# nvpro-samples/vk_gltf_renderer

Hardware: AMD Instinct MI355X
Metric: Msamples/s (and ms/frame @ fixed spp) 1080p & 4K, 1/2/4/8 MI355X (higher is better)
Workload: dtype f32

## Files before the change

vk_gltf_renderer_amd/csrc/device/mi_pt_api.hip:

```cpp
#include <hip/hip_runtime.h>

#include <algorithm>
#include <chrono>
#include <cstdlib>
#include <cmath>
#include <cstdio>
#include <cstring>
#include <memory>
#include <string>
#include <vector>

#include "mi_pt.h"
#include "bvh_refit.h"
#include "material_patch.h"
#include "pt_build.h"
#include "pt_bvh.h"
#include "pt_deform.h"
#include "pt_kernels.h"

namespace {

thread_local std::string g_lastError;

int fail(int code, const std::string& msg)
// ... 37 lines not shown
    ptr   = nullptr;
    count = 0;
  }
  ~DevBuf() { release(); }
};

enum TimedKernel { TK_GENERATE, TK_TRACE, TK_SORT, TK_SHADE, TK_SHADOW, TK_ACCUM, TK_PRIMARY, TK_SHADE_FIRST, TK_COUNT };

}

struct RunSwitches
{
  int    packetInterval = 1;
  int    sortMode       = 2;
  bool   noPacket       = false;
  bool   stateBySlot    = false;
  bool   traceSpans     = false;
  int    overlapUpTo    = 32;
  int    overlapMinTris = 200000;
  bool   noPlanes       = false;
  bool   noOpaqueTris   = false;
  bool   noQuads        = false;
  bool   shadowFarFirst = true;
  int    reinsert       = 16;
  int    reinsertUpdate = 0;
  int    reinsertRounds = 4;
  float  splitFactor    = 4.0f;
  int    splitMaxDepth  = 8;
  float  splitMinShare  = 0.1f;
  bool   collapseGreedy = false;
  bool   collapseBad    = false;
  bool   hostCollapse   = false;
  bool   coreTex        = true;
  int    maxItersDiag   = 0;
  int    failBuildAt    = 0;
  bool   candPoolSet    = false;
  size_t candPool       = 0;
  void   read()
  {
    auto flag = [](const char* n) { const char* e = getenv(n); return e != nullptr; };
    auto num  = [](const char* n, int d) { const char* e = getenv(n); return e ? atoi(e) : d; };
    packetInterval = num("MI_PT_PACKET_INTERVAL", 1);
    sortMode       = num("MI_PT_SORT", 2);
    noPacket       = flag("MI_PT_NO_PACKET");
    stateBySlot    = flag("MI_PT_STATE_BY_SLOT");
    traceSpans     = flag("MI_PT_TRACE_SPANS");
    overlapUpTo    = num("MI_PT_OVERLAP", 32);
    overlapMinTris = num("MI_PT_OVERLAP_MIN_TRIS", 200000);
    noPlanes       = flag("MI_PT_DIAG_NO_PLANES");
    noOpaqueTris   = flag("MI_PT_DIAG_NO_OPAQUE_TRIS");
    noQuads        = flag("MI_PT_DIAG_NO_QUADS");
    shadowFarFirst = num("MI_PT_SHADOW_FAR_FIRST", 1) != 0;
    reinsert       = std::max(0, num("MI_PT_REINSERT", 16));
    reinsertUpdate = std::max(0, num("MI_PT_REINSERT_UPDATE", 0));
    reinsertRounds = std::max(1, num("MI_PT_REINSERT_ROUNDS", 4));
    if(const char* e = getenv("MI_PT_SPLIT"))
      splitFactor = std::max(0.0f, float(atof(e)));
    if(const char* e = getenv("MI_PT_SPLIT_MIN_SHARE"))
      splitMinShare = std::max(0.0f, float(atof(e)));
    splitMaxDepth  = std::min(std::max(0, num("MI_PT_SPLIT_DEPTH", 8)), 10);
    if(const char* e = getenv("MI_PT_COLLAPSE"))
    {
      collapseGreedy = strcmp(e, "greedy") == 0;
      collapseBad    = !collapseGreedy && strcmp(e, "sah") != 0;
    }
    hostCollapse   = flag("MI_PT_HOST_COLLAPSE");
    maxItersDiag   = num("MI_PT_DIAG_MAX_ITERS", 0);
    coreTex        = num("MI_PT_CORE_TEX", 1) != 0;
    failBuildAt    = num("MI_PT_DIAG_FAIL_BUILD", 0);
    if(const char* e = getenv("MI_PT_DIAG_CAND_POOL"))
    {
      candPoolSet = true;
      candPool    = size_t(strtoull(e, nullptr, 10));
    }
  }
};

struct MiPt
{
  int device = 0;
  int numCUs = 256;
  RunSwitches sw;
  int accelBuilds = 0;
  int               frameQueueDepth = 1;
  int               pendingFrames   = 0;
  MiPathtraceParams pendingFirst{};
  void*             pendingStream   = nullptr;
  DevBuf<MiGltfShadeMaterial> materials;
  DevBuf<MiGltfTextureInfo>   texInfos;
  DevBuf<pt::DevTexRef>       texRefs;
  DevBuf<pt::DevCoreTex>      coreTex;
  DevBuf<MiGltfRenderNode>    nodes;
  DevBuf<pt::DevPrim>         prims;
  DevBuf<MiGltfLight>         lights;
  DevBuf<pt::DevTexture>      textures;
  DevBuf<uchar4>              texels;
  DevBuf<uint4>               texQuads;
  DevBuf<uint8_t>             geometry;
  DevBuf<uint8_t>             instFlags;
  DevBuf<float>               srgbLut;
  DevBuf<float4>              envPixels;
// ... 1869 lines not shown
  c.fc.height    = pt->height;
  c.fc.tileSize  = pt->tileSize;
  c.fc.tileShift = 0;
  while((1 << c.fc.tileShift) < pt->tileSize)
    ++c.fc.tileShift;
  c.fc.numSlots  = pt->numSlots;
  c.fc.numFrames = numFrames;
  pt::divideMagic(uint32_t(std::max(numFrames, 2)), c.fc.framesMagic, c.fc.framesShift);
  c.fc.slotLayout = numFrames % 64 == 0 ? 1 : 0;
  c.fc.stateInQueue = (!pt->sw.stateBySlot && !(pt->frameInfo.flags & MI_SCENE_INFINITE_PLANE_SHADOW_CATCHER)) ? 1 : 0;
  const bool guides = (params->flags & MI_PT_USE_OPTIX_DENOISER) != 0;
  if(int rc = ensureOptionalPathArrays(pt, c.fc.stateInQueue == 0, params->numSamples > 1, guides, (pt->frameInfo.flags & MI_SCENE_INFINITE_PLANE_SHADOW_CATCHER) != 0))
    return rc;
  c.paths        = pt->paths;
  {
    const bool stateBySlot = c.fc.stateInQueue == 0, multiSample = params->numSamples > 1;
    if(!(stateBySlot || multiSample))
      c.paths.misc = nullptr;
    if(!stateBySlot)
      c.paths.throughput = nullptr;
    if(!multiSample)
      c.paths.pixelSum = nullptr;
  }
  pt->accumFrames   = float(params->totalSamples) / float(params->numSamples) + float(numFrames);
  if(guides && (params->totalSamples == 0 || pt->momentFrames == pt->accumFrames - float(numFrames)))
    pt->momentFrames = pt->accumFrames;
  else if(!guides || params->totalSamples == 0)
    pt->momentFrames = 0.0f;
  if(!guides)
  {
    c.paths.guideAlbedo = nullptr;
    c.paths.guideNormal = nullptr;
  }
  c.queues           = pt->queues;
  if(!(pt->frameInfo.flags & MI_SCENE_INFINITE_PLANE_SHADOW_CATCHER))
    c.queues.shadow.aux2 = nullptr;
  c.ownedTiles       = pt->ownedTiles.ptr;
  c.stats            = pt->stats.ptr;
  c.stream           = stream;
  c.persistentBlocks = unsigned(pt->numCUs) * 8u;
  c.hasAlpha         = pt->hasAlpha;
  c.hasAlphaClosest  = c.hasAlpha && pt->hasAlphaTest;
  c.visualization    = pt->frameInfo.visualization > MI_VIZ_RENDERED && pt->frameInfo.visualization < MI_VIZ_COUNT;
  if(pt->frameInfo.visualization == MI_VIZ_OPACITY_MICROMAP)
    c.hasAlphaClosest = false;
  c.hasTransmissive  = pt->hasTransmissive;
  c.simpleMaterials  = pt->simpleMaterials;
  c.wide             = pt->wide;
  c.collectCounters  = pt->collectCounters;
  {
    c.sortMode = pt->sw.sortMode;
  }
  if(pt->sceneDevDirty)
  {
    HIP_TRY(hipDeviceSynchronize());
    HIP_TRY(pt->sceneDev.upload(&pt->scene, 1));
    pt->sceneDevDirty = false;
  }
  if(!pt->fcHost)
  {
    HIP_TRY(hipHostMalloc(reinterpret_cast<void**>(&pt->fcHost), sizeof(pt::FrameConsts) * MiPt::FC_RING, hipHostMallocDefault));
    HIP_TRY(pt->fcRing.alloc(MiPt::FC_RING));
    for(hipEvent_t& e : pt->fcDone)
      HIP_TRY(hipEventCreateWithFlags(&e, hipEventDisableTiming));
  }
  const unsigned fcSlot = pt->fcCursor++ % unsigned(MiPt::FC_RING);
// ... 654 lines not shown
```

vk_gltf_renderer_amd/csrc/device/pt_kernels.hip:

```cpp
#include <hip/hip_runtime.h>
#include <hip/hip_fp16.h>

#ifndef MI_PT_EXACT_FP
#define PT_FAST_SHADING_MATH 1
#endif
#include "pt_kernels.h"
#include "pt_shading.h"
#include "pt_bvh.h"
#include "pt_bvh8.h"
#include "pt_packet.h"
#include "pt_feed.h"
#include "pt_visualize.h"

namespace pt {

namespace {

constexpr int TRACE_BLOCK = 1024;
#ifndef NODE_CACHE_EXTRA
#define NODE_CACHE_EXTRA 0
#endif
constexpr int NODE_CACHE  = 712 + NODE_CACHE_EXTRA;
constexpr int NODE_CACHE_ALPHA = 504 + NODE_CACHE_EXTRA;
constexpr int SEL_BLOCK   = 256;
// ... 305 lines not shown
    const uint32_t pos   = (chunk % NSUB) * Q.subCap + (chunk / NSUB) * QCHUNK + (slot % QCHUNK);
    Q.active[0].slot[pos] = cp.valid ? slot : QUEUE_DEAD;
    if(cp.valid)
    {
      Q.active[0].org[pos] = make_float4(cp.origin.x, cp.origin.y, cp.origin.z, 0.0f);
      Q.active[0].dir[pos] = make_float4(cp.direction.x, cp.direction.y, cp.direction.z, __uint_as_float(cp.seed));
      if(fc.stateInQueue)
        Q.active[0].misc[pos] = make_float4(0.0f, __uint_as_float(PF_ALIVE), __uint_as_float(cp.seed), 0.0f);
    }
  }
  if(blockIdx.x == 0 && threadIdx.x < NSUB)
  {
    const uint32_t numChunks = batchSlots / QCHUNK;
    Q.counters[QC_PAIR0 + 2 * threadIdx.x] = QCHUNK * (numChunks / NSUB + (threadIdx.x < numChunks % NSUB ? 1u : 0u));
  }
  if(blockIdx.x == 0 && threadIdx.x < 8)
    Q.counters[QC_HEADS_TRACE + threadIdx.x] = 0;
  (void)sc;
}

#ifdef TRACE_PROFILE
__device__ unsigned long long g_traceProf[20];
__device__ unsigned long long g_shadowProf[16];
#define PROF_T() __builtin_amdgcn_s_memtime()
#define PROF_ADD(i, t0) profAcc[i] += PROF_T() - (t0)
#define PROF_CNT(i, n) profCnt[i] += (unsigned long long)(n)
#else
#define PROF_T() 0ull
#define PROF_ADD(i, t0) (void)(t0)
#define PROF_CNT(i, n) (void)0
#endif

#ifdef SHADE_PROFILE
__device__ unsigned long long g_shadeProf[20];
#define SPROF_BEGIN() const unsigned long long sprofT0_ = __builtin_amdgcn_s_memtime(); const int sprofLanes_ = __popcll(__ballot(true))
#define SPROF_END(r)                                                                                                             \
  do                                                                                                                             \
  {                                                                                                                              \
    if(!FIRST)                                                                                                                   \
    {                                                                                                                            \
      const unsigned long long dt_ = __builtin_amdgcn_s_memtime() - sprofT0_;                                                   \
      if(laneId() == uint32_t(__ffsll((long long)__ballot(true)) - 1))                                                          \
      {                                                                                                                          \
        atomicAdd(&g_shadeProf[2 * (r)], dt_);                                                                                   \
        atomicAdd(&g_shadeProf[2 * (r) + 1], dt_ * (unsigned long long)sprofLanes_);                                             \
      }                                                                                                                          \
    }                                                                                                                            \
  } while(0)
#else
#define SPROF_BEGIN() (void)0
#define SPROF_END(r) (void)0
#endif

#ifndef REFILL_IDLE_LANES
#define REFILL_IDLE_LANES 16
#endif
#ifndef TRI_PHASE_LANES_N
#define TRI_PHASE_LANES_N 24
#endif
constexpr int TRI_PHASE_LANES      = TRI_PHASE_LANES_N;
constexpr int TRI_PHASE_EXIT_LANES = 10;
#ifndef TRI_ROUND_LANES
#define TRI_ROUND_LANES 20
#endif
#ifndef TRI_ROUND_LANE_CAP_N
#define TRI_ROUND_LANE_CAP_N 4
#endif
// ... 1723 lines not shown
    out[i] = makeShadeRecord(sc, sc.tris[i]);
}

__global__ void __launch_bounds__(256) k_texture_quads(const uint32_t* __restrict__ texels, uint4* __restrict__ quads, uint32_t offset, int w, int h, int wrapS, int wrapT)
{
  const uint32_t i = blockIdx.x * 256u + threadIdx.x;
  if(i >= uint32_t(w) * uint32_t(h))
    return;
  const int x = int(i % uint32_t(w)), y = int(i / uint32_t(w));
  const int x1 = wrapS == MI_WRAP_CLAMP_TO_EDGE ? min(x + 1, w - 1) : (x + 1 == w ? 0 : x + 1);
  const int y1 = wrapT == MI_WRAP_CLAMP_TO_EDGE ? min(y + 1, h - 1) : (y + 1 == h ? 0 : y + 1);
  const uint32_t* L = texels + offset;
  quads[offset + i] = make_uint4(L[uint32_t(y) * uint32_t(w) + uint32_t(x)], L[uint32_t(y) * uint32_t(w) + uint32_t(x1)],
                                 L[uint32_t(y1) * uint32_t(w) + uint32_t(x)], L[uint32_t(y1) * uint32_t(w) + uint32_t(x1)]);
}

__global__ void k_reset_counters(uint32_t* counters)
{
  for(int i = threadIdx.x; i < QC_COUNT; i += blockDim.x)
    counters[i] = 0;
}

}

void launchBuildAlphaRecords(const DevScene& scene, uint32_t numTris, DevAlphaTri* out, hipStream_t s)
{
  if(numTris)
    hipLaunchKernelGGL(k_alpha_records, dim3((numTris + 255) / 256), dim3(256), 0, s, scene, numTris, out);
}
void dumpTraceProfile()
{
#ifdef SHADE_PROFILE
  {
    unsigned long long h[20] = {};
    (void)hipDeviceSynchronize();
    (void)hipMemcpyFromSymbol(h, HIP_SYMBOL(g_shadeProf), sizeof(h));
    const double tot = h[18] ? double(h[18]) : 1.0;
    const char*  names[9] = {"entry + hit state", "material + textures", "sampleLights", "bsdfEvaluate", "bsdfSample", "(unused)", "miss (inline / listed)", "append + stores", "finishMisses"};
    fprintf(stderr, "[mi_pt shade profile] later-bounce k_shade: round ticks %.4g, lanes with an entry %.1f\n", tot, h[18] ? double(h[19]) / double(h[18]) : 0.0);
    for(int r = 0; r < 9; ++r)
      if(h[2 * r])
        fprintf(stderr, "[mi_pt shade profile]   %-24s %5.1f %% of the round's wave time, %5.1f lanes inside\n", names[r], 100.0 * double(h[2 * r]) / tot,
                r == 8 ? 0.0 : double(h[2 * r + 1]) / double(h[2 * r]));
  }
#endif
#ifdef TRACE_PROFILE
  unsigned long long h[20] = {};
  (void)hipDeviceSynchronize();
  (void)hipMemcpyFromSymbol(h, HIP_SYMBOL(g_traceProf), sizeof(h));
  const double tot = double(h[3]) > 0 ? double(h[3]) : 1.0;
  fprintf(stderr, "[mi_pt trace profile] feed split: start-ray (waits for the prefetch) %.1f%% take %.1f%% issue %.1f%%\n", 100.0 * h[5] / tot, 100.0 * h[6] / tot,
          100.0 * h[7] / tot);
  fprintf(stderr, "[mi_pt trace profile] waves %llu total ticks %.4g: feed %.1f%% node %.1f%% tri %.1f%% other %.1f%%\n", h[4], tot, 100.0 * h[0] / tot,
          100.0 * h[1] / tot, 100.0 * h[2] / tot, 100.0 * (tot - h[0] - h[1] - h[2]) / tot);
  fprintf(stderr, "[mi_pt trace profile] triangle rounds: test (permutes, intersection, alpha) %.1f%% gather %.1f%% of total; alpha rounds %.1f%% of total (%llu rounds)\n",
          100.0 * h[16] / tot, 100.0 * h[17] / tot, 100.0 * h[18] / tot, h[19]);
  unsigned long long g[16] = {};
  (void)hipMemcpyFromSymbol(g, HIP_SYMBOL(g_shadowProf), sizeof(g));
  const double st = double(g[5]) > 0 ? double(g[5]) : 1.0;
  const auto   pr = [](unsigned long long a, unsigned long long b) { return b ? double(a) / double(b) : 0.0; };
  fprintf(stderr, "[mi_pt shadow profile] waves %llu total ticks %.4g: feed %.1f%% node %.1f%% tri %.1f%% alpha %.1f%% finish %.1f%% other %.1f%%\n", g[6], st,
          100.0 * g[0] / st, 100.0 * g[1] / st, 100.0 * g[2] / st, 100.0 * g[3] / st, 100.0 * g[4] / st, 100.0 * (st - g[0] - g[1] - g[2] - g[3] - g[4]) / st);
  fprintf(stderr, "[mi_pt shadow profile] outer iterations %llu (%.1f idle lanes each), inner iterations %llu (%.1f active lanes, %.1f visiting), alpha rounds %llu (%.1f entries)\n",
          g[8], pr(g[9], g[8]), g[10], pr(g[11], g[10]), pr(g[12], g[10]), g[13], pr(g[14], g[13]));
  const auto per = [](unsigned long long a, unsigned long long b) { return b ? double(a) / double(b) : 0.0; };
  fprintf(stderr, "[mi_pt trace profile] lanes: %.1f of 64 visit per node step (%llu steps, %.1f blocked); %.1f test per triangle round (%llu rounds in %llu phases); "
                  "%.1f idle at each of %llu refills\n",
          per(h[9], h[8]), h[8], per(h[15], h[8]), per(h[11], h[10]), h[10], h[14], per(h[13], h[12]), h[12]);
#endif
// ... 193 lines not shown
```

vk_gltf_renderer_amd/csrc/device/pt_scene.h:

```cpp
#pragma once
#include <hip/hip_runtime.h>
#include <stdint.h>

#include "mi_pt.h"
#include "pt_math.h"

namespace pt {

struct DevTexture
{
  uint32_t levelOffset[16];
  uint16_t width, height;
  uint8_t  numLevels;
  uint8_t  srgb;
  uint8_t  magFilter, minFilter, mipmapMode, wrapS, wrapT;
  uint8_t  _pad[5];
};

struct DevTexRef
{
  float    uv[6];
  uint32_t level0;
  uint16_t width, height;
  uint8_t  numLevels, srgb, magFilter, minFilter, mipmapMode, wrapS, wrapT, texCoord;
// ... 111 lines not shown
  const float*               srgbLut;
  int                        numMaterials, numTextures, numLights, numNodes;
  int                        envWidth, envHeight;
  int                        numTris;
  int                        bvh8NumNodes;
  int                        bvhRoot;
  int                        packetInterval;
  uint32_t                   shadowOctFlip;
};

struct SkyPrecomp
{
  float sunDir[3], cosS;
  float thetaS, tS, T, cosTs;
  float sunE[3], Yz;
  float xz, yz, sunRadius, coneAngle;
  float coneOneMinusCos, omega, denY, denX;
  float denYy, pad0, pad1, pad2;
  float cY[5], cX[5], cYy[5], pad3;
};
struct FrameConsts
{
  MiSceneFrameInfo        frameInfo;
  MiSkyPhysicalParameters sky;
  const SkyPrecomp*       skyPre;
  MiPathtraceParams       pc;
  int                     width, height;
  int                     tileSize, tileShift;
  int                     numSlots;
  int                     numFrames;
  uint32_t                framesMagic, framesShift;
  int                     slotLayout;
  int                     stateInQueue;
};

inline void divideMagic(uint32_t d, uint32_t& magic, uint32_t& shift)
{
  uint32_t k = 31;
  while(!(d >> k))
    --k;
  if((d & (d - 1u)) == 0u)
  {
    magic = 0x80000000u;
    shift = k - 1u;
    return;
  }
  const unsigned long long p = 1ull << (32 + k);
  magic                      = uint32_t((p + d - 1ull) / d);
  shift                      = k;
}

#if defined(__HIPCC__)
template <class T, class I>
__device__ __forceinline__ const T& gat(const T* table, I i)
{
  return *(const T*)((const __attribute__((address_space(1))) T*)table + i);
}
template <class T>
__device__ __forceinline__ const T& uniformConst(const T& r)
{
  const unsigned long long p = reinterpret_cast<unsigned long long>(&r);
  const uint32_t           lo = uint32_t(__builtin_amdgcn_readfirstlane(int(uint32_t(p)))), hi = uint32_t(__builtin_amdgcn_readfirstlane(int(uint32_t(p >> 32))));
  const unsigned long long u  = (unsigned long long)lo | ((unsigned long long)hi << 32);
  return *(const T*)(const __attribute__((address_space(4))) T*)u;
}
#else
// ... 109 lines not shown
```

vk_gltf_renderer_amd/csrc/device/pt_shade_body.h:

```cpp
  const DevScene&    sc = uniformConst(*scp);
  const FrameConsts& fc = uniformConst(*fcp);
  const bool         stateInQueue = fc.stateInQueue != 0;
  __shared__ uint32_t s_prefix[NSUB + 1];
  __shared__ uint32_t s_push[4];
  __shared__ float    s_srgb[256];
#ifndef SHADE_NO_DEFERRED_MISS
  constexpr bool DEFER_MISS = !FIRST;
#else
  constexpr bool DEFER_MISS = false;
#endif
  __shared__ uint32_t s_missPos[DEFER_MISS ? 2 * SHADE_BLOCK : 1];
  __shared__ uint32_t s_missCount;
  const bool          deferMiss = DEFER_MISS && !hasFlag(fc.frameInfo.flags, MI_SCENE_USE_INFINITE_PLANE) && !hasFlag(fc.frameInfo.flags, MI_SCENE_USE_HDR_ENVIRONMENT);
  if(threadIdx.x == 0)
    s_missCount = 0;
  auto finishMisses = [&](bool all) {
    __syncthreads();
    const uint32_t n = s_missCount;
    if(n == 0u || (!all && n < uint32_t(SHADE_BLOCK)))
      return;
    const uint32_t take = min(n, uint32_t(SHADE_BLOCK)), base = n - take;
    uint32_t       pos = 0;
    if(threadIdx.x < take)
      pos = s_missPos[base + threadIdx.x];
// ... 139 lines not shown
    {
      SPROF_BEGIN();
      const float4 hit4 = Q.active[cur].aux[inPos], o4 = Q.active[cur].org[inPos], d4 = Q.active[cur].dir[inPos];
      const float4 misc4 = stateInQueue ? Q.active[cur].misc[inPos] : P.misc[slot];
      const float4 tp4   = FIRST ? make_float4(1.0f, 1.0f, 1.0f, DIRAC) : (stateInQueue ? Q.active[cur].aux2[inPos] : P.throughput[slot]);
      const float4 rad4  = FIRST ? make_float4(0.0f, 0.0f, 0.0f, 0.0f) : (stateInQueue ? Q.active[cur].rad[inPos] : P.radiance[slot]);
      f3       rayOrigin = xyz(o4), rayDir = xyz(d4);
      float    coneWidth = misc4.w;
      f3       throughput = xyz(tp4), radiance = xyz(rad4);
      float    lastSamplePdf = tp4.w;
      f2       maxRoughness  = mk2(fabsf(rad4.w), misc4.x);
      uint32_t flags = __float_as_uint(misc4.y), seed = __float_as_uint(misc4.z);
      int      surfaceDepth   = int((flags >> PF_DEPTH_SHIFT) & 0xffu);
      int      scatterBounces = int((flags >> PF_SCATTER_SHIFT) & 0xffu);
      bool     isInside = !SIMPLE && (flags & PF_INSIDE) != 0u, solid = !(flags & PF_NOT_SOLID);
      const bool firstRay = (surfaceDepth == 0);
      bool       guideWritten = false;
      const int  maxDepth = fc.pc.maxDepth;
      const bool needFirstHit = hasFlag(fc.pc.flags, MI_PT_FIRST_FRAME) && pathSlotFrame(fc, slot) == 0u;

      float hitT   = hit4.x;
      int   triIdx = __float_as_int(hit4.y);
      bool  done   = false;
      bool  deferred = false;
      bool  earlyContinue = false;

      HitState hit;
      uint4    core0 = make_uint4(0u, 0u, 0u, 0u);
      int      rnodeID = -1, primitiveID = -1, materialID = 0;
      (void)primitiveID;
      int      rprimID = -1, ommState = 0;
      bool     frontFace = true;
      const bool meshHit = triIdx >= 0;
      if(meshHit)
      {
        const DevShadeTri S = gat(sc.shadeTris, triIdx);
        rnodeID             = int(S.rnode);
        primitiveID         = int(S.prim);
        materialID          = S.materialID;
        if(!FIRST)
          core0 = gat(sc.coreTex, 5u * uint32_t(materialID));
        const MiGltfRenderNode& rn = gat(sc.nodes, rnodeID);
        DevPrim rp{};
        u3      ti{0u, 0u, 0u};
        if(S.attrs & (SHADE_HAS_UV1 | SHADE_HAS_COLORS))
        {
          rp = gat(sc.prims, S.renderPrimID);
          ti = getTriangleIndices(rp, int(S.prim));
        }
        hit = getHitState(&gat(sc.geomPool, S.v0), &gat(sc.geomPool, S.v1), &gat(sc.geomPool, S.v2), S.attrs, &rp, ti,
                          mk3(1.0f - hit4.z - hit4.w, hit4.z, hit4.w), rn.worldToObject, rn.objectToWorld, rayDir, VIZ ? &frontFace : nullptr);
        if(P.firstHitTri && firstRay && needFirstHit)
          P.firstHitTri[pathSlotPixel(fc, slot)] = make_uint4(uint32_t(S.renderPrimID), S.prim, __float_as_uint(hit4.z), __float_as_uint(hit4.w));
        if constexpr(VIZ)
        {
          rprimID = S.renderPrimID;
          if(fc.frameInfo.visualization == MI_VIZ_OPACITY_MICROMAP)
            ommState = (__float_as_uint(gat(sc.tris, triIdx).c.w) & INST_FORCE_OPAQUE) ? 0 : 1;
        }
      }
      else
        hitT = INFINITE_F;
      SPROF_END(0);

      bool hitInfinitePlane = false;
      {
        const float t = infinitePlaneT(fc, rayOrigin, rayDir, hitT);
// ... 16 lines not shown
        s_missPos[atomicAdd(&s_missCount, 1u)] = inPos;
        deferred = true;
        done     = true;
        SPROF_END(6);
      }
      else if(hitT == INFINITE_F)
      {
        SPROF_BEGIN();
        bool backplate = false;
        if(firstRay)
        {
          solid             = false;
          if(needFirstHit)
            P.firstHit[pathSlotPixel(fc, slot)] = make_float4(rayDir.x, rayDir.y, rayDir.z, 0.0f);
          backplate = primaryMissBackplate(sc, fc, rayDir, radiance);
        }
        if(!backplate)
        {
          f3    envColor;
          float mis;
          missEnvironment(sc, fc, rayDir, lastSamplePdf, envColor, mis);
          radiance += throughput * mis * envColor;
        }
        done = true;
        SPROF_END(6);
      }

      if(!done)
      {
        PbrMaterial pbrMat;
        float worldFoot = (coneWidth + fc.pc.pixelAngle * hitT) / fmaxf(fabsf(dot(hit.geonrm, -rayDir)), 1e-3f);
        bool  unlit     = false;
        bool  catcherPlane = false;
        if(hitInfinitePlane)
        {
          pbrMat           = defaultPbrMaterial();
          pbrMat.baseColor = mk3(fc.frameInfo.infinitePlaneBaseColor);
          pbrMat.metallic  = fc.frameInfo.infinitePlaneMetallic;
          float r          = fc.frameInfo.infinitePlaneRoughness;
          pbrMat.roughness = mk2(r * r, r * r);
          pbrMat.N = hit.nrm; pbrMat.Ng = hit.nrm; pbrMat.Nc = hit.nrm;
          pbrMat.T = hit.tangent; pbrMat.B = hit.bitangent;
          if(hasFlag(fc.frameInfo.flags, MI_SCENE_INFINITE_PLANE_SHADOW_CATCHER))
          {
            catcherPlane = true;
            coneWidth    = worldFoot;
            if(FIRST && needFirstHit)
              P.firstHit[pathSlotPixel(fc, slot)] = make_float4(1e34f, 1e34f, 1e34f, __uint_as_float(TEMPORAL_ID_INVALID));
            DirectLight dl;
            sampleLights(sc, fc, hit.pos, seed, dl);
            const bool traceIt = dot(dl.direction, hit.nrm) > 0.0f && dl.pdf != 0.0f;
            f3         envColor;
            float      envPdf;
            sampleEnvironment(sc, fc, rayDir, envColor, envPdf);
            const float mis         = computeEnvHitMisWeight(sc, fc, lastSamplePdf, envPdf);
            const f3    unshadowed  = throughput * mis * envColor;
            if(!traceIt)
            {
              radiance += unshadowed;
              done = true;
            }
            else
            {
              shOrg = make_float4(hit.pos.x, hit.pos.y, hit.pos.z, INFINITE_F);
              shDir = make_float4(dl.direction.x, dl.direction.y, dl.direction.z, __uint_as_float(2u));
              shCon = make_float4(envColor.x, envColor.y, envColor.z, __uint_as_float(seed));
              shCon2     = make_float4(unshadowed.x, unshadowed.y, unshadowed.z, 0.0f);
// ... 300 lines not shown
```

vk_gltf_renderer_amd/csrc/device/pt_shading.h:

```cpp
#pragma once
#include <cstddef>

#include "pt_light.h"

namespace pt {

constexpr float MIN_TRANSMISSION                = 0.01f;
constexpr float ANTIALIASING_STANDARD_DEVIATION = 0.4246609f;
constexpr int   RR_MIN_DEPTH                    = 3;
constexpr float VOLUME_MIN_SCATTER              = 0.001f;
constexpr float VOLUME_RAND_FLOOR               = 1.0e-10f;
constexpr int   VOLUME_FREE_BUDGET              = 64;
constexpr float RR_PCONT_FLOOR                  = 0.001f;
constexpr float RR_PCONT_CAP                    = 0.95f;
constexpr float MICROFACET_MIN_ROUGHNESS        = 0.0014142f;

PT_DEV bool hasFlag(int flags, int f) { return (flags & f) != 0; }

struct u3
{
  uint32_t x, y, z;
};
PT_DEV u3 getTriangleIndices(const DevPrim& rp, int prim)
{
// ... 230 lines not shown
}
PT_DEV float texLod(const float* U, float texGrad, float W, float H)
{
#pragma clang fp contract(off)
  const float ax = (U[0] * texGrad) * W, bx = (U[1] * texGrad) * H, ay = (U[2] * texGrad) * W, by = (U[3] * texGrad) * H;
  return texLodOf(__fmaf_rn(bx, bx, ax * ax), __fmaf_rn(by, by, ay * ay));
}
PT_DEV float texLodIdentity(float texGrad, float W, float H)
{
#pragma clang fp contract(off)
  const float ax = texGrad * W, by = texGrad * H;
  return texLodOf(ax * ax, by * by);
}
PT_DEV DevTexRef loadTexRef(const DevTexRef* refs, uint32_t slot)
{
#if !defined(__HIPCC__)
  return refs[slot];
#else
  typedef uint32_t u32x4 __attribute__((ext_vector_type(4)));
  typedef uint32_t u32x3 __attribute__((ext_vector_type(3)));
  const DevTexRef* p = refs + slot;
  u32x4            a, b;
  u32x3            c;
  asm volatile("global_load_dwordx4 %0, %3, off\n\tglobal_load_dwordx4 %1, %3, off offset:16\n\tglobal_load_dwordx3 %2, %3, off offset:32\n\ts_waitcnt vmcnt(0)"
               : "=&v"(a), "=&v"(b), "=&v"(c)
               : "v"(p)
               : "memory");
  DevTexRef R;
  uint32_t* W = reinterpret_cast<uint32_t*>(&R);
  W[0] = a[0]; W[1] = a[1]; W[2] = a[2]; W[3] = a[3]; W[4] = b[0]; W[5] = b[1]; W[6] = b[2]; W[7] = b[3]; W[8] = c[0]; W[9] = c[1]; W[10] = c[2];
  return R;
#endif
}
__device__ __noinline__ f4 getTextureRef(TexCtx tc, uint32_t slot, f2 tc0, f2 tc1, float texGrad)
{
#ifdef MI_PT_DIAG_NO_TEX
  return mk4(0.5f + 1e-3f * (tc0.x + tc1.y + texGrad + float(slot)));
#endif
  const DevTexRef R  = loadTexRef(tc.refs, slot);
  f2              t  = R.texCoord == 0 ? tc0 : tc1;
  const float*    U  = R.uv;
  f2              uv = texUv(U, t);
  if(R.width == 0)
    return mk4(1.0f);
  float lod = 0.0f;
  if(texGrad > 0.0f)
    lod = texLod(U, texGrad, float(R.width), float(R.height));
  if(lod <= 0.0f)
    return sampleLevelRef(tc, R, uv, 0, R.magFilter);
  float maxLevel = float(int(R.numLevels) - 1);
  lod            = fminf(lod, maxLevel);
  if(R.mipmapMode == MI_FILTER_NEAREST)
    return sampleLevelRef(tc, R, uv, min(int(floorf(lod + 0.5f)), int(R.numLevels) - 1), R.minFilter);
  int   l0 = int(floorf(lod)), l1 = min(l0 + 1, int(R.numLevels) - 1);
  float f  = lod - float(l0);
  if(R.minFilter != MI_FILTER_NEAREST && hasQuadPath(tc, R) && !(f == 0.0f || l1 == l0))
  {
    const uint32_t off0 = levelOffsetRef(R, l0), off1 = off0 + uint32_t(max(1, int(R.width) >> l0)) * uint32_t(max(1, int(R.height) >> l0));
    const QuadTap  t0 = quadTap(R, uv, l0, off0), t1 = quadTap(R, uv, l1, off1);
    const uint4   q0 = gat(tc.quads, t0.index), q1 = gat(tc.quads, t1.index);
    const f4      a = quadFilter(tc, R, t0, q0), b = quadFilter(tc, R, t1, q1);
    return levelBlend(a, b, f);
  }
  f4    a  = sampleLevelRef(tc, R, uv, l0, R.minFilter);
  if(f == 0.0f || l1 == l0)
    return a;
  f4 b = sampleLevelRef(tc, R, uv, l1, R.minFilter);
  return levelBlend(a, b, f);
}
#ifndef MI_PT_CORE_TEX_BATCH
#define MI_PT_CORE_TEX_BATCH 1
#endif
struct CoreTap
{
  uint32_t i0, i1;
  float    tx0, ty0, tx1, ty1, f;
  uint32_t bits;
};
enum : uint32_t { CP_FAST = 1u, CP_TWO = 2u, CP_SRGB = 4u, CP_DUPX0 = 8u, CP_DUPY0 = 16u, CP_DUPX1 = 32u, CP_DUPY1 = 64u, CP_SLOW = 128u };
PT_DEV CoreTap coreTexPlan(const TexCtx& tc, const uint4 c, f2 tc0, f2 tc1, float texGrad)
{
  CoreTap p;
  p.i0 = p.i1 = 0u;
  p.tx0 = p.ty0 = p.tx1 = p.ty1 = p.f = 0.0f;
  p.bits = 0u;
  const int W = int(c.y & 0xffffu), H = int(c.y >> 16);
  if(W == 0)
    return p;
#ifdef MI_PT_DIAG_NO_TEX
  p.bits = CP_SLOW;
  return p;
#endif
  if(!(c.z & CT_FAST) || !tc.quads)
  {
    p.bits = CP_SLOW;
    return p;
  }
  const f2 t   = (c.z & CT_TEXCOORD1) ? tc1 : tc0;
  f2       uv  = t;
  float    lod = 0.0f;
  if(c.z & CT_TRANSFORM)
  {
// ... 50 lines not shown
  if(p.bits & CP_SLOW)
    return getTextureRef(tc, slot, tc0, tc1, texGrad);
  if(!(p.bits & CP_FAST))
    return mk4(1.0f);
  const bool srgb = (p.bits & CP_SRGB) != 0u;
  const f4   a    = quadFilterS(tc, srgb, p.tx0, p.ty0, (p.bits & CP_DUPX0) != 0u, (p.bits & CP_DUPY0) != 0u, q0);
  if(!(p.bits & CP_TWO))
    return a;
  const f4 b = quadFilterS(tc, srgb, p.tx1, p.ty1, (p.bits & CP_DUPX1) != 0u, (p.bits & CP_DUPY1) != 0u, q1);
  return levelBlend(a, b, p.f);
}
PT_DEV f3 multiToSingleScatterAlbedo(f3 rho)
{
  f3 t = mk3(4.09712f) + rho * 4.20863f - sqrt3(mk3(9.59217f) + rho * 41.6808f + rho * rho * 17.7126f);
  return mk3(1.0f) - t * t;
}
PT_DEV f3 convertSGToMR(f3 diffuseColor, f3 specularColor, float glossiness, float& metallic, f2& roughness)
{
  const float dielectricSpecular = 0.04f;
  float       specularIntensity  = fmaxf(specularColor.x, fmaxf(specularColor.y, specularColor.z));
  metallic                       = smoothstepf(dielectricSpecular + 0.01f, dielectricSpecular + 0.05f, specularIntensity);
  f3 baseColor;
  if(metallic > 0.0f)
    baseColor = specularColor;
  else
  {
    baseColor = diffuseColor / (1.0f - dielectricSpecular * (1.0f - metallic));
    baseColor = clamp3(baseColor, 0.0f, 1.0f);
  }
  float r   = 1.0f - glossiness;
  roughness = mk2(r * r, r * r);
  return baseColor;
}
template <bool SIMPLE, bool CORE = false>
PT_DEV PbrMaterial evaluateMaterial(const DevScene& sc, const MiGltfShadeMaterial& m, const MeshState& st, unsigned& taps)
{
#define TEX(slot) (++taps, getTextureRef(st.tex, slot, st.tc0, st.tc1, st.texGrad))
  PbrMaterial p = defaultPbrMaterial();
  static_assert(offsetof(MiGltfShadeMaterial, pbrBaseColorTexture) % 8 == 0 && offsetof(MiGltfShadeMaterial, occlusionTexture) == offsetof(MiGltfShadeMaterial, pbrBaseColorTexture) + 8,
                "core texture slots: base colour, normal, metallic-roughness, emissive, occlusion");
  const uint32_t* slotWords = reinterpret_cast<const uint32_t*>(&m.pbrBaseColorTexture);
  const uint32_t  sw0 = slotWords[0], sw1 = slotWords[1], sw2 = slotWords[2];
  const uint16_t  texBaseColor = uint16_t(sw0 & 0xffffu), texNormal = uint16_t(sw0 >> 16), texMetallicRoughness = uint16_t(sw1 & 0xffffu),
                 texEmissive = uint16_t(sw1 >> 16), texOcclusion = uint16_t(sw2 & 0xffffu);
  CoreTap cp0{};
  uint4   cq0 = make_uint4(0u, 0u, 0u, 0u), cq1 = cq0;
  if(CORE && MI_PT_CORE_TEX_BATCH)
  {
    const bool  present = m.pbrModel != MI_PBR_SPECULAR_GLOSSINESS && isTexturePresent(texBaseColor);
    const uint4 c       = st.core0;
    cp0                 = coreTexPlan(st.tex, present ? c : make_uint4(0u, 0u, 0u, 0u), st.tc0, st.tc1, st.texGrad);
    coreTexIssue(st.tex, cp0, cq0, cq1);
  }
  if(m.pbrModel == MI_PBR_SPECULAR_GLOSSINESS)
  {
    f4    diffuse    = mk4(m.pbrDiffuseFactor[0], m.pbrDiffuseFactor[1], m.pbrDiffuseFactor[2], m.pbrDiffuseFactor[3]) * st.baseColorVertexMul;
    float glossiness = m.pbrGlossinessFactor;
    f3    specular   = mk3(m.pbrSpecularFactor);
    if(isTexturePresent(m.pbrDiffuseTexture))
      diffuse *= TEX(m.pbrDiffuseTexture);
    if(isTexturePresent(m.pbrSpecularGlossinessTexture))
    {
      f4 s = TEX(m.pbrSpecularGlossinessTexture);
      specular *= xyz(s);
      glossiness *= s.w;
    }
    p.baseColor = convertSGToMR(xyz(diffuse), specular, glossiness, p.metallic, p.roughness);
    p.opacity   = diffuse.w;
  }
  else
  {
    f4 baseColor = mk4(m.pbrBaseColorFactor[0], m.pbrBaseColorFactor[1], m.pbrBaseColorFactor[2], m.pbrBaseColorFactor[3]) * st.baseColorVertexMul;
    if(isTexturePresent(texBaseColor))
      baseColor *= (CORE && MI_PT_CORE_TEX_BATCH) ? (++taps, coreTexFinish(st.tex, cp0, cq0, cq1, texBaseColor, st.tc0, st.tc1, st.texGrad)) : TEX(texBaseColor);
    p.baseColor     = xyz(baseColor);
    p.opacity       = baseColor.w;
    float roughness = m.pbrRoughnessFactor, metallic = m.pbrMetallicFactor;
    if(isTexturePresent(texMetallicRoughness))
    {
      f4 s = TEX(texMetallicRoughness);
      roughness *= s.y;
      metallic *= s.z;
    }
    roughness   = fmaxf(roughness, MICROFACET_MIN_ROUGHNESS);
    p.roughness = mk2(roughness * roughness, roughness * roughness);
    p.metallic  = clampf(metallic, 0.0f, 1.0f);
  }
  p.occlusion = m.occlusionStrength;
  if(isTexturePresent(texOcclusion))
  {
    float occ   = TEX(texOcclusion).x;
    p.occlusion = 1.0f + p.occlusion * (occ - 1.0f);
  }
  p.N  = st.N;
  p.T  = st.T;
  p.B  = st.B;
  p.Ng = st.Ng;
  bool needsTangentUpdate = false;
  if(isTexturePresent(texNormal))
  {
    f3 nv = xyz(TEX(texNormal));
    nv    = nv * 2.0f - mk3(1.0f);
    nv *= mk3(m.normalTextureScale, m.normalTextureScale, 1.0f);
    p.N                = normalize(st.T * nv.x + st.B * nv.y + st.N * nv.z);
    needsTangentUpdate = true;
  }
  p.emissive = mk3(m.emissiveFactor);
  if(isTexturePresent(texEmissive))
    p.emissive *= xyz(TEX(texEmissive));
  p.emissive            = max3(mk3(0.0f), p.emissive);
  if(!SIMPLE)
  {
    p.attenuationColor    = mk3(m.attenuationColor);
    p.attenuationDistance = m.attenuationDistance;
    p.thickness           = m.thicknessFactor;
    if(isTexturePresent(m.thicknessTexture))
      p.thickness *= TEX(m.thicknessTexture).y;
  }
  p.specularColor = mk3(m.specularColorFactor);
  if(isTexturePresent(m.specularColorTexture))
    p.specularColor *= xyz(TEX(m.specularColorTexture));
  p.specular = m.specularFactor;
  if(isTexturePresent(m.specularTexture))
    p.specular *= TEX(m.specularTexture).w;
  float ior1 = 1.0f, ior2 = m.ior;
  if(!SIMPLE && st.isInside && (p.thickness > 0.0f))
  {
    ior1 = ior2;
    ior2 = 1.0f;
  }
  p.ior1         = ior1;
  p.ior2         = ior2;
  bool needsTangentUpdateAniso = false;
  if(!SIMPLE)
  {
  p.transmission = m.transmissionFactor;
  if(isTexturePresent(m.transmissionTexture))
    p.transmission *= TEX(m.transmissionTexture).x;
  f3 ms = mk3(m.multiscatterColorFactor);
  if(ms.x > 0.0f || ms.y > 0.0f || ms.z > 0.0f)
  {
    f3 ssa               = multiToSingleScatterAlbedo(ms);
    f3 attC              = -log3(max3(p.attenuationColor, mk3(0.001f))) / fmaxf(p.attenuationDistance, 0.001f);
    p.scatterCoefficient = attC * ssa;
  }
  p.scatterAnisotropy  = m.scatterAnisotropy;
  p.clearcoat          = m.clearcoatFactor;
  p.clearcoatRoughness = m.clearcoatRoughness;
  p.Nc                 = p.N;
  if(isTexturePresent(m.clearcoatTexture))
    p.clearcoat *= TEX(m.clearcoatTexture).x;
  if(isTexturePresent(m.clearcoatRoughnessTexture))
    p.clearcoatRoughness *= TEX(m.clearcoatRoughnessTexture).y;
  if(isTexturePresent(m.clearcoatNormalTexture))
  {
    f3 nv = xyz(TEX(m.clearcoatNormalTexture));
    nv    = nv * 2.0f - mk3(1.0f);
    p.Nc  = normalize(p.T * nv.x + p.B * nv.y + p.Nc * nv.z);
  }
  p.clearcoatRoughness = fmaxf(p.clearcoatRoughness, 0.001f);
  float iridescence = m.iridescenceFactor, iridescenceThickness = m.iridescenceThicknessMaximum;
  p.iridescenceIor = m.iridescenceIor;
  if(isTexturePresent(m.iridescenceTexture))
    iridescence *= TEX(m.iridescenceTexture).x;
  if(isTexturePresent(m.iridescenceThicknessTexture))
  {
    float t              = TEX(m.iridescenceThicknessTexture).y;
    iridescenceThickness = lerpf(m.iridescenceThicknessMinimum, m.iridescenceThicknessMaximum, t);
  }
  p.iridescence          = (iridescenceThickness > 0.0f) ? iridescence : 0.0f;
  p.iridescenceThickness = iridescenceThickness;
  float anisotropyStrength = m.anisotropyStrength;
  if(anisotropyStrength > 0.0f)
  {
    f2 dir = mk2(1.0f, 0.0f);
    if(isTexturePresent(m.anisotropyTexture))
    {
      f4 a = TEX(m.anisotropyTexture);
      dir  = normalize(mk2(a.x, a.y) * 2.0f - mk2(1.0f, 1.0f));
      anisotropyStrength *= a.z;
    }
    p.roughness.x = lerpf(p.roughness.y, 1.0f, anisotropyStrength * anisotropyStrength);
    float s = m.anisotropyRotation[0], c = m.anisotropyRotation[1];
    dir                = mk2(c * dir.x + s * dir.y, c * dir.y - s * dir.x);
    p.T                = p.T * dir.x + p.B * dir.y;
    needsTangentUpdateAniso = true;
  }
  }
  needsTangentUpdate = needsTangentUpdate || needsTangentUpdateAniso;
  if(needsTangentUpdate)
  {
    p.B         = normalize(cross(p.N, p.T));
    float bsign = signfz(dot(st.B, p.B));
    p.B         = p.B * bsign;
    p.T         = normalize(cross(p.B, p.N) * bsign);
  }
  if(!SIMPLE)
  {
  p.sheenColor = mk3(m.sheenColorFactor);
  if(isTexturePresent(m.sheenColorTexture))
    p.sheenColor *= xyz(TEX(m.sheenColorTexture));
  p.sheenRoughness = m.sheenRoughnessFactor;
  if(isTexturePresent(m.sheenRoughnessTexture))
    p.sheenRoughness *= TEX(m.sheenRoughnessTexture).w;
  p.sheenRoughness            = fmaxf(MICROFACET_MIN_ROUGHNESS, p.sheenRoughness);
  p.dispersion                = m.dispersion;
  p.diffuseTransmissionFactor = m.diffuseTransmissionFactor;
  if(isTexturePresent(m.diffuseTransmissionTexture))
    p.diffuseTransmissionFactor *= TEX(m.diffuseTransmissionTexture).w;
  p.diffuseTransmissionColor = mk3(m.diffuseTransmissionColor);
  if(isTexturePresent(m.diffuseTransmissionColorTexture))
    p.diffuseTransmissionColor *= xyz(TEX(m.diffuseTransmissionColorTexture));
  p.retroreflection = m.retroreflectionFactor;
  if(isTexturePresent(m.retroreflectionTexture))
    p.retroreflection *= TEX(m.retroreflectionTexture).x;
  }
#undef TEX
  return p;
}

PT_DEV f3 safeOffsetRay(f3 p, f3 dir)
{
  const float scaleValue = 256.0f;
  int         ix = int(scaleValue * dir.x), iy = int(scaleValue * dir.y), iz = int(scaleValue * dir.z);
  f3 op = mk3(__int_as_float(__float_as_int(p.x) + ((p.x < 0) ? -ix : ix)), __int_as_float(__float_as_int(p.y) + ((p.y < 0) ? -iy : iy)),
              __int_as_float(__float_as_int(p.z) + ((p.z < 0) ? -iz : iz)));
  const float origin = 1.0f / 32.0f, floatScale = 1.0f / 65536.0f;
  return mk3(fabsf(p.x) < origin ? p.x + floatScale * dir.x : op.x, fabsf(p.y) < origin ? p.y + floatScale * dir.y : op.y,
             fabsf(p.z) < origin ? p.z + floatScale * dir.z : op.z);
}

PT_DEV float getOpacityFast(const DevScene& sc, int triIndex, f3 bary)
{
  const DevAlphaTri rec  = sc.alphaTris[triIndex];
  const uint32_t    flg  = rec.c.z;
  const uint32_t    mode = flg & AT_MODE_MASK;
  if(mode == MI_ALPHA_OPAQUE)
    return 1.0f;
  float alpha = rec.b.z;
  if(flg & AT_HAS_TEXTURE)
  {
    f2          uv = mk2(rec.a.x, rec.a.y) * bary.x + mk2(rec.a.z, rec.a.w) * bary.y + mk2(rec.b.x, rec.b.y) * bary.z;
    const int   w = int(rec.c.y & 0xffffu), h = int(rec.c.y >> 16);
    const int   wrapS = int((flg >> AT_WRAPS_SHIFT) & 3u), wrapT = int((flg >> AT_WRAPT_SHIFT) & 3u);
    const uchar4* texels = sc.texels + rec.c.x;
    float       fx = uv.x * float(w), fy = uv.y * float(h);
    float       ta;
    if(!(flg & AT_LINEAR))
      ta = float(texels[texelIndex(0u, w, wrapCoord(int(floorf(fx)), w, wrapS), wrapCoord(int(floorf(fy)), h, wrapT))].w) * (1.0f / 255.0f);
    else
// ... 344 lines not shown
```

Baseline: 749.5.

## Add wave-uniform first-bounce shading path with scalar triangle and material loads

For first-bounce shading, the kernel detects when every active lane of a wave hit the same triangle. In that case it loads the triangle record, node transform, vertices, material and texture references through readfirstlane and uniform (scalar) loads instead of per-lane vector gathers. Material texture slots are read as uniform 32-bit words so the compiler can keep them in scalar registers. This aims to cut vector memory traffic and VGPR pressure on coherent primary hits, at the cost of an extra ballot check per wave and a larger code footprint.

Result: no change. 752.7 (median of 3 runs) (+0.4%).

```diff
diff --git a/vk_gltf_renderer_amd/csrc/device/mi_pt_api.hip b/vk_gltf_renderer_amd/csrc/device/mi_pt_api.hip
--- a/vk_gltf_renderer_amd/csrc/device/mi_pt_api.hip
+++ b/vk_gltf_renderer_amd/csrc/device/mi_pt_api.hip
@@ -93,6 +93,7 @@
   bool   collapseBad    = false;
   bool   hostCollapse   = false;
   bool   coreTex        = true;
+  bool   uniformShade   = true;
   int    maxItersDiag   = 0;
   int    failBuildAt    = 0;
   bool   candPoolSet    = false;
@@ -128,6 +129,7 @@
     hostCollapse   = flag("MI_PT_HOST_COLLAPSE");
     maxItersDiag   = num("MI_PT_DIAG_MAX_ITERS", 0);
     coreTex        = num("MI_PT_CORE_TEX", 1) != 0;
+    uniformShade   = num("MI_PT_UNIFORM_SHADE", 1) != 0;
     failBuildAt    = num("MI_PT_DIAG_FAIL_BUILD", 0);
     if(const char* e = getenv("MI_PT_DIAG_CAND_POOL"))
     {
@@ -2063,6 +2065,7 @@
     c.paths.guideAlbedo = nullptr;
     c.paths.guideNormal = nullptr;
   }
+  c.fc.uniformShade  = (pt->sw.uniformShade && c.fc.slotLayout == 1 && !(pt->frameInfo.flags & MI_SCENE_USE_INFINITE_PLANE) && !c.paths.firstHitTri) ? 1 : 0;
   c.queues           = pt->queues;
   if(!(pt->frameInfo.flags & MI_SCENE_INFINITE_PLANE_SHADOW_CATCHER))
     c.queues.shadow.aux2 = nullptr;
diff --git a/vk_gltf_renderer_amd/csrc/device/pt_kernels.hip b/vk_gltf_renderer_amd/csrc/device/pt_kernels.hip
--- a/vk_gltf_renderer_amd/csrc/device/pt_kernels.hip
+++ b/vk_gltf_renderer_amd/csrc/device/pt_kernels.hip
@@ -361,7 +361,7 @@
 #endif
 
 #ifdef SHADE_PROFILE
-__device__ unsigned long long g_shadeProf[20];
+__device__ unsigned long long g_shadeProf[22];
 #define SPROF_BEGIN() const unsigned long long sprofT0_ = __builtin_amdgcn_s_memtime(); const int sprofLanes_ = __popcll(__ballot(true))
 #define SPROF_END(r)                                                                                                             \
   do                                                                                                                             \
@@ -2151,9 +2151,11 @@
 {
 #ifdef SHADE_PROFILE
   {
-    unsigned long long h[20] = {};
+    unsigned long long h[22] = {};
     (void)hipDeviceSynchronize();
     (void)hipMemcpyFromSymbol(h, HIP_SYMBOL(g_shadeProf), sizeof(h));
+    if(h[20] + h[21])
+      fprintf(stderr, "[mi_pt shade profile] bounce-0 k_shade: %llu waves with a live lane, %llu of them uniform (%.1f %%)\n", h[20] + h[21], h[20], 100.0 * double(h[20]) / double(h[20] + h[21]));
     const double tot = h[18] ? double(h[18]) : 1.0;
     const char*  names[9] = {"entry + hit state", "material + textures", "sampleLights", "bsdfEvaluate", "bsdfSample", "(unused)", "miss (inline / listed)", "append + stores", "finishMisses"};
     fprintf(stderr, "[mi_pt shade profile] later-bounce k_shade: round ticks %.4g, lanes with an entry %.1f\n", tot, h[18] ? double(h[19]) / double(h[18]) : 0.0);
diff --git a/vk_gltf_renderer_amd/csrc/device/pt_scene.h b/vk_gltf_renderer_amd/csrc/device/pt_scene.h
--- a/vk_gltf_renderer_amd/csrc/device/pt_scene.h
+++ b/vk_gltf_renderer_amd/csrc/device/pt_scene.h
@@ -167,6 +167,7 @@
   uint32_t                framesMagic, framesShift;
   int                     slotLayout;
   int                     stateInQueue;
+  int                     uniformShade;
 };
 
 inline void divideMagic(uint32_t d, uint32_t& magic, uint32_t& shift)
diff --git a/vk_gltf_renderer_amd/csrc/device/pt_shade_body.h b/vk_gltf_renderer_amd/csrc/device/pt_shade_body.h
--- a/vk_gltf_renderer_amd/csrc/device/pt_shade_body.h
+++ b/vk_gltf_renderer_amd/csrc/device/pt_shade_body.h
@@ -195,7 +195,33 @@
       int      rprimID = -1, ommState = 0;
       bool     frontFace = true;
       const bool meshHit = triIdx >= 0;
-      if(meshHit)
+      bool     uniformWave = false;
+      uint32_t uniformTri  = 0u;
+      if constexpr(FIRST && !VIZ)
+      {
+        if(fc.uniformShade != 0)
+        {
+          uniformTri  = uint32_t(__builtin_amdgcn_readfirstlane(triIdx));
+          uniformWave = int(uniformTri) >= 0 && __ballot(uint32_t(triIdx) == uniformTri) == __ballot(true)
+                        && !(uniformConst(gat(sc.shadeTris, uniformTri)).attrs & (SHADE_HAS_UV1 | SHADE_HAS_COLORS));
+        }
+#ifdef SHADE_PROFILE
+        if(laneId() == uint32_t(__ffsll((long long)__ballot(true)) - 1))
+          atomicAdd(&g_shadeProf[uniformWave ? 20 : 21], 1ull);
+#endif
+      }
+      if(uniformWave)
+      {
+        const DevShadeTri& S = uniformConst(gat(sc.shadeTris, uniformTri));
+        rnodeID              = int(S.rnode);
+        primitiveID          = int(S.prim);
+        materialID           = S.materialID;
+        const MiGltfRenderNode& rn = uniformConst(gat(sc.nodes, S.rnode));
+        hit = getHitState(&uniformConst(gat(sc.geomPool, S.v0)), &uniformConst(gat(sc.geomPool, S.v1)), &uniformConst(gat(sc.geomPool, S.v2)),
+                          S.attrs & ~uint32_t(SHADE_HAS_UV1 | SHADE_HAS_COLORS), nullptr, u3{0u, 0u, 0u},
+                          mk3(1.0f - hit4.z - hit4.w, hit4.z, hit4.w), rn.worldToObject, rn.objectToWorld, rayDir, nullptr);
+      }
+      else if(meshHit)
       {
         const DevShadeTri S = gat(sc.shadeTris, triIdx);
         rnodeID             = int(S.rnode);
@@ -278,7 +304,21 @@
         float worldFoot = (coneWidth + fc.pc.pixelAngle * hitT) / fmaxf(fabsf(dot(hit.geonrm, -rayDir)), 1e-3f);
         bool  unlit     = false;
         bool  catcherPlane = false;
-        if(hitInfinitePlane)
+        if(uniformWave)
+        {
+          const MiGltfShadeMaterial& mat = uniformConst(gat(sc.materials, __builtin_amdgcn_readfirstlane(materialID)));
+          MeshState                  mesh;
+          mesh.N = hit.nrm; mesh.T = hit.tangent; mesh.B = hit.bitangent; mesh.Ng = hit.geonrm;
+          mesh.tc0 = hit.uv0; mesh.tc1 = hit.uv1;
+          mesh.isInside           = isInside;
+          mesh.texGrad            = worldFoot * hit.texelDensity * fc.pc.texGradScale;
+          mesh.baseColorVertexMul = hit.color;
+          mesh.tex                = TexCtx{sc.texRefs, sc.texels, s_srgb, sc.texQuads};
+          mesh.core0              = core0;
+          pbrMat                  = evaluateMaterial<SIMPLE, false, true>(sc, mat, mesh, taps);
+          unlit                   = mat.unlit > 0;
+        }
+        else if(hitInfinitePlane)
         {
           pbrMat           = defaultPbrMaterial();
           pbrMat.baseColor = mk3(fc.frameInfo.infinitePlaneBaseColor);
diff --git a/vk_gltf_renderer_amd/csrc/device/pt_shading.h b/vk_gltf_renderer_amd/csrc/device/pt_shading.h
--- a/vk_gltf_renderer_amd/csrc/device/pt_shading.h
+++ b/vk_gltf_renderer_amd/csrc/device/pt_shading.h
@@ -286,12 +286,8 @@
   return R;
 #endif
 }
-__device__ __noinline__ f4 getTextureRef(TexCtx tc, uint32_t slot, f2 tc0, f2 tc1, float texGrad)
-{
-#ifdef MI_PT_DIAG_NO_TEX
-  return mk4(0.5f + 1e-3f * (tc0.x + tc1.y + texGrad + float(slot)));
-#endif
-  const DevTexRef R  = loadTexRef(tc.refs, slot);
+PT_DEV f4 textureOfRef(const TexCtx& tc, const DevTexRef& R, f2 tc0, f2 tc1, float texGrad)
+{
   f2              t  = R.texCoord == 0 ? tc0 : tc1;
   const float*    U  = R.uv;
   f2              uv = texUv(U, t);
@@ -322,6 +318,28 @@
   f4 b = sampleLevelRef(tc, R, uv, l1, R.minFilter);
   return levelBlend(a, b, f);
 }
+__device__ __noinline__ f4 getTextureRef(TexCtx tc, uint32_t slot, f2 tc0, f2 tc1, float texGrad)
+{
+#ifdef MI_PT_DIAG_NO_TEX
+  return mk4(0.5f + 1e-3f * (tc0.x + tc1.y + texGrad + float(slot)));
+#endif
+  const DevTexRef R = loadTexRef(tc.refs, slot);
+  return textureOfRef(tc, R, tc0, tc1, texGrad);
+}
+__device__ __noinline__ f4 getTextureRefUniform(TexCtx tc, uint32_t slot, f2 tc0, f2 tc1, float texGrad)
+{
+#ifdef MI_PT_DIAG_NO_TEX
+  return mk4(0.5f + 1e-3f * (tc0.x + tc1.y + texGrad + float(slot)));
+#endif
+  const uint32_t* w = reinterpret_cast<const uint32_t*>(&uniformConst(gat(tc.refs, slot)));
+  static_assert(sizeof(DevTexRef) == 44, "11 words");
+  DevTexRef       R;
+  uint32_t*       W = reinterpret_cast<uint32_t*>(&R);
+#pragma unroll
+  for(int i = 0; i < 11; ++i)
+    W[i] = w[i];
+  return textureOfRef(tc, R, tc0, tc1, texGrad);
+}
 #ifndef MI_PT_CORE_TEX_BATCH
 #define MI_PT_CORE_TEX_BATCH 1
 #endif
@@ -438,10 +456,23 @@
   roughness = mk2(r * r, r * r);
   return baseColor;
 }
-template <bool SIMPLE, bool CORE = false>
+template <bool UNIFORM>
+PT_DEV uint16_t materialSlot(const MiGltfShadeMaterial& m, const uint16_t& field)
+{
+  if constexpr(!UNIFORM)
+    return field;
+  else
+  {
+    const size_t   off = size_t(reinterpret_cast<const char*>(&field) - reinterpret_cast<const char*>(&m));
+    const uint32_t w   = reinterpret_cast<const uint32_t*>(&m)[off >> 2];
+    return uint16_t((off & 2u) ? (w >> 16) : (w & 0xffffu));
+  }
+}
+template <bool SIMPLE, bool CORE = false, bool UNIFORM = false>
 PT_DEV PbrMaterial evaluateMaterial(const DevScene& sc, const MiGltfShadeMaterial& m, const MeshState& st, unsigned& taps)
 {
-#define TEX(slot) (++taps, getTextureRef(st.tex, slot, st.tc0, st.tc1, st.texGrad))
+#define SLOT(f) materialSlot<UNIFORM>(m, m.f)
+#define TEX(slot) (++taps, UNIFORM ? getTextureRefUniform(st.tex, slot, st.tc0, st.tc1, st.texGrad) : getTextureRef(st.tex, slot, st.tc0, st.tc1, st.texGrad))
   PbrMaterial p = defaultPbrMaterial();
   static_assert(offsetof(MiGltfShadeMaterial, pbrBaseColorTexture) % 8 == 0 && offsetof(MiGltfShadeMaterial, occlusionTexture) == offsetof(MiGltfShadeMaterial, pbrBaseColorTexture) + 8,
                 "core texture slots: base colour, normal, metallic-roughness, emissive, occlusion");
@@ -463,11 +494,11 @@
     f4    diffuse    = mk4(m.pbrDiffuseFactor[0], m.pbrDiffuseFactor[1], m.pbrDiffuseFactor[2], m.pbrDiffuseFactor[3]) * st.baseColorVertexMul;
     float glossiness = m.pbrGlossinessFactor;
     f3    specular   = mk3(m.pbrSpecularFactor);
-    if(isTexturePresent(m.pbrDiffuseTexture))
-      diffuse *= TEX(m.pbrDiffuseTexture);
-    if(isTexturePresent(m.pbrSpecularGlossinessTexture))
+    if(isTexturePresent(SLOT(pbrDiffuseTexture)))
+      diffuse *= TEX(SLOT(pbrDiffuseTexture));
+    if(isTexturePresent(SLOT(pbrSpecularGlossinessTexture)))
     {
-      f4 s = TEX(m.pbrSpecularGlossinessTexture);
+      f4 s = TEX(SLOT(pbrSpecularGlossinessTexture));
       specular *= xyz(s);
       glossiness *= s.w;
     }
@@ -520,15 +551,15 @@
     p.attenuationColor    = mk3(m.attenuationColor);
     p.attenuationDistance = m.attenuationDistance;
     p.thickness           = m.thicknessFactor;
-    if(isTexturePresent(m.thicknessTexture))
-      p.thickness *= TEX(m.thicknessTexture).y;
+    if(isTexturePresent(SLOT(thicknessTexture)))
+      p.thickness *= TEX(SLOT(thicknessTexture)).y;
   }
   p.specularColor = mk3(m.specularColorFactor);
-  if(isTexturePresent(m.specularColorTexture))
-    p.specularColor *= xyz(TEX(m.specularColorTexture));
+  if(isTexturePresent(SLOT(specularColorTexture)))
+    p.specularColor *= xyz(TEX(SLOT(specularColorTexture)));
   p.specular = m.specularFactor;
-  if(isTexturePresent(m.specularTexture))
-    p.specular *= TEX(m.specularTexture).w;
+  if(isTexturePresent(SLOT(specularTexture)))
+    p.specular *= TEX(SLOT(specularTexture)).w;
   float ior1 = 1.0f, ior2 = m.ior;
   if(!SIMPLE && st.isInside && (p.thickness > 0.0f))
   {
@@ -541,8 +572,8 @@
   if(!SIMPLE)
   {
   p.transmission = m.transmissionFactor;
-  if(isTexturePresent(m.transmissionTexture))
-    p.transmission *= TEX(m.transmissionTexture).x;
+  if(isTexturePresent(SLOT(transmissionTexture)))
+    p.transmission *= TEX(SLOT(transmissionTexture)).x;
   f3 ms = mk3(m.multiscatterColorFactor);
   if(ms.x > 0.0f || ms.y > 0.0f || ms.z > 0.0f)
   {
@@ -554,24 +585,24 @@
   p.clearcoat          = m.clearcoatFactor;
   p.clearcoatRoughness = m.clearcoatRoughness;
   p.Nc                 = p.N;
-  if(isTexturePresent(m.clearcoatTexture))
-    p.clearcoat *= TEX(m.clearcoatTexture).x;
-  if(isTexturePresent(m.clearcoatRoughnessTexture))
-    p.clearcoatRoughness *= TEX(m.clearcoatRoughnessTexture).y;
-  if(isTexturePresent(m.clearcoatNormalTexture))
-  {
-    f3 nv = xyz(TEX(m.clearcoatNormalTexture));
+  if(isTexturePresent(SLOT(clearcoatTexture)))
+    p.clearcoat *= TEX(SLOT(clearcoatTexture)).x;
+  if(isTexturePresent(SLOT(clearcoatRoughnessTexture)))
+    p.clearcoatRoughness *= TEX(SLOT(clearcoatRoughnessTexture)).y;
+  if(isTexturePresent(SLOT(clearcoatNormalTexture)))
+  {
+    f3 nv = xyz(TEX(SLOT(clearcoatNormalTexture)));
     nv    = nv * 2.0f - mk3(1.0f);
     p.Nc  = normalize(p.T * nv.x + p.B * nv.y + p.Nc * nv.z);
   }
   p.clearcoatRoughness = fmaxf(p.clearcoatRoughness, 0.001f);
   float iridescence = m.iridescenceFactor, iridescenceThickness = m.iridescenceThicknessMaximum;
   p.iridescenceIor = m.iridescenceIor;
-  if(isTexturePresent(m.iridescenceTexture))
-    iridescence *= TEX(m.iridescenceTexture).x;
-  if(isTexturePresent(m.iridescenceThicknessTexture))
-  {
-    float t              = TEX(m.iridescenceThicknessTexture).y;
+  if(isTexturePresent(SLOT(iridescenceTexture)))
+    iridescence *= TEX(SLOT(iridescenceTexture)).x;
+  if(isTexturePresent(SLOT(iridescenceThicknessTexture)))
+  {
+    float t              = TEX(SLOT(iridescenceThicknessTexture)).y;
     iridescenceThickness = lerpf(m.iridescenceThicknessMinimum, m.iridescenceThicknessMaximum, t);
   }
   p.iridescence          = (iridescenceThickness > 0.0f) ? iridescence : 0.0f;
@@ -580,9 +611,9 @@
   if(anisotropyStrength > 0.0f)
   {
     f2 dir = mk2(1.0f, 0.0f);
-    if(isTexturePresent(m.anisotropyTexture))
+    if(isTexturePresent(SLOT(anisotropyTexture)))
     {
-      f4 a = TEX(m.anisotropyTexture);
+      f4 a = TEX(SLOT(anisotropyTexture));
       dir  = normalize(mk2(a.x, a.y) * 2.0f - mk2(1.0f, 1.0f));
       anisotropyStrength *= a.z;
     }
@@ -604,24 +635,25 @@
   if(!SIMPLE)
   {
   p.sheenColor = mk3(m.sheenColorFactor);
-  if(isTexturePresent(m.sheenColorTexture))
-    p.sheenColor *= xyz(TEX(m.sheenColorTexture));
+  if(isTexturePresent(SLOT(sheenColorTexture)))
+    p.sheenColor *= xyz(TEX(SLOT(sheenColorTexture)));
   p.sheenRoughness = m.sheenRoughnessFactor;
-  if(isTexturePresent(m.sheenRoughnessTexture))
-    p.sheenRoughness *= TEX(m.sheenRoughnessTexture).w;
+  if(isTexturePresent(SLOT(sheenRoughnessTexture)))
+    p.sheenRoughness *= TEX(SLOT(sheenRoughnessTexture)).w;
   p.sheenRoughness            = fmaxf(MICROFACET_MIN_ROUGHNESS, p.sheenRoughness);
   p.dispersion                = m.dispersion;
   p.diffuseTransmissionFactor = m.diffuseTransmissionFactor;
-  if(isTexturePresent(m.diffuseTransmissionTexture))
-    p.diffuseTransmissionFactor *= TEX(m.diffuseTransmissionTexture).w;
+  if(isTexturePresent(SLOT(diffuseTransmissionTexture)))
+    p.diffuseTransmissionFactor *= TEX(SLOT(diffuseTransmissionTexture)).w;
   p.diffuseTransmissionColor = mk3(m.diffuseTransmissionColor);
-  if(isTexturePresent(m.diffuseTransmissionColorTexture))
-    p.diffuseTransmissionColor *= xyz(TEX(m.diffuseTransmissionColorTexture));
+  if(isTexturePresent(SLOT(diffuseTransmissionColorTexture)))
+    p.diffuseTransmissionColor *= xyz(TEX(SLOT(diffuseTransmissionColorTexture)));
   p.retroreflection = m.retroreflectionFactor;
-  if(isTexturePresent(m.retroreflectionTexture))
-    p.retroreflection *= TEX(m.retroreflectionTexture).x;
+  if(isTexturePresent(SLOT(retroreflectionTexture)))
+    p.retroreflection *= TEX(SLOT(retroreflectionTexture)).x;
   }
 #undef TEX
+#undef SLOT
   return p;
 }
 
```
